# Lacadame/DiffSci

Hardware: AMD Instinct MI355X
Metric: samples/sec (50-step Karras Heun), PUNetG 64ch 128x128 (higher is better)
Workload: dtype f32 (3x3 convs: fp16 hi+lo split, 3 fp16 MFMA products, fp32 accumulate); 1 GPU; PUNetG 64-base-ch, 1x128x128 fields, batch 64 per GPU, 50-step Heun deterministic sampler (99 network evaluations); global_batch=64, parallelism=dp1 (batch shards, all-gather of samples), world_size=1, backend=none (one process), hipgraph=True

## Files before the change

### build.py

```python
#!/usr/bin/env python3
import os
import subprocess
import sys

ROOT = os.path.dirname(os.path.abspath(__file__))
CSRC = os.path.join(ROOT, "diffsci_amd", "csrc")
OUTDIR = os.path.join(ROOT, "diffsci_amd", "_lib")
LIB = os.path.join(OUTDIR, "libdiffsci_hip.so")
SOURCES = ["ds_api.hip", "ds_step.hip", "ds_ddpm.hip", "ds_inpaint.hip", "ds_norm.hip", "ds_gnorm.hip", "ds_normtab.hip", "ds_conv.hip", "ds_conv6.hip", "ds_conv3h.hip", "ds_conv3p.hip", "ds_convup.hip", "ds_conv1h.hip", "ds_conv_s2.hip", "ds_convdirect.hip", "ds_conv3d.hip", "ds_resample.hip", "ds_attn.hip", "ds_attn3h.hip", "ds_small.hip", "ds_amax.hip", "ds_tokens.hip", "ds_convit.hip", "ds_groupnorm.hip", "ds_window.hip", "ds_periodize.hip"]
HIPCC = os.environ.get("HIPCC", "/opt/rocm/bin/hipcc")
FLAGS = ["--offload-arch=gfx950", "-O3", "-ffp-contract=off", "-fPIC", "-std=c++17",
         "-Wall", "-Wno-unused-function"] + os.environ.get("DS_EXTRA_HIPCC_FLAGS", "").split()
EXTRA_FLAGS = {f: ["-fno-slp-vectorize"] for f in ("ds_conv3h.hip", "ds_conv3p.hip", "ds_convup.hip", "ds_conv1h.hip", "ds_conv_s2.hip")}
EXTRA_FLAGS["ds_conv3p.hip"] = EXTRA_FLAGS["ds_conv3p.hip"] + ["-Wno-inline-asm"]


def _stale():
    if not os.path.exists(LIB):
        return True
    t = os.path.getmtime(LIB)
    deps = [os.path.join(CSRC, f) for f in os.listdir(CSRC)] + [os.path.join(ROOT, "include", "diffsci_hip.h"), os.path.abspath(__file__)]
    return any(os.path.getmtime(d) > t for d in deps)


def build(force=False, verbose=True):
    os.makedirs(OUTDIR, exist_ok=True)
    if not force and not _stale():
        return LIB
    objs = []
    procs = []
    for src in SOURCES:
        obj = os.path.join(OUTDIR, src.replace(".hip", ".o"))
        cmd = [HIPCC] + FLAGS + EXTRA_FLAGS.get(src, []) + ["-c", os.path.join(CSRC, src), "-o", obj]
        if verbose:
            print(" ".join(cmd), flush=True)
        procs.append((src, subprocess.Popen(cmd)))
        objs.append(obj)
    for src, p in procs:
        if p.wait() != 0:
            raise RuntimeError(f"hipcc failed on {src}")
    cmd = [HIPCC, "--offload-arch=gfx950", "-shared", "-fPIC", "-o", LIB] + objs
    if verbose:
        print(" ".join(cmd), flush=True)
    subprocess.check_call(cmd)
    return LIB

# ... 4 lines not shown
```

### diffsci_amd/csrc/ds_conv1h.hip

```cpp
#include "ds_common.h"
#include "ds_conv_epilogue.h"
#include "ds_h3_common.h"

namespace {

using ds_epi::f32x16;
using ds_h3::f16x8;
using ds_h3::split2;
using ds_h3::u32x4;
typedef const __attribute__((address_space(1))) float* gfloat_ptr;
typedef const __attribute__((address_space(1))) char* gchar_ptr;
typedef float f32x2 __attribute__((ext_vector_type(2)));
typedef const __attribute__((address_space(1))) f32x2* gfloat2_ptr;

constexpr int COT = 64, NT = 256, KC = 16;
constexpr int NPOS = 256;
constexpr int XBUF_VEC = 2 * 2 * NPOS;
constexpr int WSLAB_VEC = 2 * 2 * COT;
constexpr int NXB = 3, NWS = 3;
constexpr int RING_BYTES = (NXB * XBUF_VEC + NWS * WSLAB_VEC) * 16;
constexpr int EPI_BYTES = 4 * 64 * 2 * 32 * 4;
constexpr int STAGE_BYTES = RING_BYTES > EPI_BYTES ? RING_BYTES : EPI_BYTES;
constexpr int LDS_BYTES = STAGE_BYTES + 128 * 4;
constexpr int TWO_RING_BYTES = (NXB * XBUF_VEC + NWS * 2 * WSLAB_VEC) * 16;
constexpr int TWO_EPI_BYTES = 8 * 64 * 2 * 32 * 4;
static_assert(TWO_EPI_BYTES >= TWO_RING_BYTES, "bias / shift rows behind the larger of the two");
constexpr int LDS_BYTES_TWO = TWO_EPI_BYTES + 2 * 128 * 4;
constexpr int NXCD = 8;

struct Conv1hArgs {
  float* out;
  const float* in;
  const u32x4* wp;
  const float* bias;
  const float* shift;
  const float* res1;
  const float* res2;
  float* tile_stats;
  int res1_up;
  const unsigned* in_amax;
  unsigned* out_amax;
  int wshift;
  int amax_split;
  int shift_stride;
  int B, Cin, Cout, H, W, Hin, Win;
  int tiles_x, tiles_y, n_cot, n_chunks;
  int n_cot_wg;
  unsigned n_blocks;
};

__device__ __forceinline__ void step_barrier() {
  asm volatile("s_waitcnt lgkmcnt(0)\n\ts_barrier" ::: "memory");
}

template <int MODE, bool W16, bool TWO = false>
__global__ __launch_bounds__(TWO ? 2 * NT : NT, 2) void k_conv1h(const Conv1hArgs a) {
  constexpr int TW = W16 ? 16 : 32, TH = W16 ? 16 : 8;
  constexpr int COTS = TWO ? 2 : 1;
  constexpr int KR = TWO ? KC / 2 : KC;
  extern __shared__ __attribute__((aligned(16))) unsigned char smem[];
  u32x4* Xs = reinterpret_cast<u32x4*>(smem);
  u32x4* Ws = Xs + NXB * XBUF_VEC;
  float* BS = reinterpret_cast<float*>(smem + (TWO ? TWO_EPI_BYTES : STAGE_BYTES));
  const int tid = threadIdx.x;
  const int lane = tid & 63;
  const int wv = __builtin_amdgcn_readfirstlane(tid >> 6);
  const int cw = TWO ? wv >> 2 : 0;
  const int wq = wv & 3;
  const int pix = tid & (NT - 1);
  const int li = lane & 31, lh = lane >> 5;

  unsigned bid;
  {
    const unsigned x = blockIdx.x % NXCD, k = blockIdx.x / NXCD;
    const unsigned per = a.n_blocks / NXCD, rem = a.n_blocks % NXCD;
    bid = x * per + (x < rem ? x : rem) + k;
// ... 96 lines not shown
  x_fetch(R1, n > 1 ? 1 : 0);
  __builtin_amdgcn_sched_barrier(0);
  ascale = ds_epi::act_scale_of(amax_bits, a.wshift);
  w_store(W0, 0);
  x_store(R0, 0);
  ds_epi::commit_bias_shift(BS, bias_shift, COTS);
  __syncthreads();

  int buf = 0;
  auto step = [&](float (&Ra)[KR], u32x4& Wa, float (&Rb)[KR], u32x4& Wb, int g) {
    const int gf = g + 2 < n ? g + 2 : n - 1;
    w_fetch(Wa, gf);
    x_fetch(Ra, gf);
    mma(g % NWS, buf);
    const int nb = buf == NXB - 1 ? 0 : buf + 1;
    w_store(Wb, (g + 1) % NWS);
    x_store(Rb, nb);
    buf = nb;
    step_barrier();
  };
  int g = 0;
  for (; g + 1 < n; g += 2) {
    step(R0, W0, R1, W1, g);
    step(R1, W1, R0, W0, g + 1);
  }
  if (g < n) step(R0, W0, R1, W1, g);
  __syncthreads();

  {
    ds_epi::Args e;
    e.out = a.out; e.bias = a.bias; e.shift = a.shift; e.res1 = a.res1; e.res2 = a.res2; e.res1_up = a.res1_up;
    e.unscale = ds_epi::unscale_from_in(ascale.in_scale, a.wshift); e.shift_stride = a.shift_stride;
    e.out_amax = a.out_amax ? a.out_amax + b + ((a.amax_split > 0 && (cot + cw) * COT >= a.amax_split) ? a.B : 0) : nullptr;
    e.b = b; e.co_base = (cot + cw) * COT; e.y0 = y0 + (W16 ? 4 : 2) * wq; e.x0 = x0;
    e.Cout = a.Cout; e.H = a.H; e.W = a.W;
    e.tile_stats = a.tile_stats; e.tile = ty * a.tiles_x + tx; e.ntiles = a.tiles_x * a.tiles_y;
    float* tile = reinterpret_cast<float*>(smem) + wv * (64 * 2 * 32);
    ds_epi::store_tile<W16>(acc, tile, BS + 128 * cw, e);
    if (a.tile_stats) {
      __syncthreads();
      if constexpr (TWO) {
        if (tid < 128) {
          e.co_base = (cot + (tid >> 6)) * COT;
          ds_epi::store_tile_stats(reinterpret_cast<const float*>(smem) + (tid >> 6) * 4 * (64 * 2 * 32), 64 * 2 * 32, e, tid & 63);
        }
      } else {
        ds_epi::store_tile_stats(reinterpret_cast<const float*>(smem), 64 * 2 * 32, e);
      }
    }
  }
}

__global__ void k_pack1h(_Float16* packed, const float* __restrict__ w, int Cout, int Cin, int n_chunks, float scale,
                         size_t total) {
  size_t i = (size_t)blockIdx.x * blockDim.x + threadIdx.x;
  if (i >= total) return;
  size_t t = i;
  const int c8 = t % 8; t /= 8;
  const int co64 = t % COT; t /= COT;
  const int h = t % 2; t /= 2;
  const int piece = t % 2; t /= 2;
  const int chunk = t % n_chunks; t /= n_chunks;
  const int cot = (int)t;
  const int co = cot * COT + co64, ci = chunk * KC + 8 * h + c8;
  float v = 0.f;
  if (co < Cout && ci < Cin) v = w[(size_t)co * Cin + ci] * scale;
  const _Float16 hi = (_Float16)v;
  const _Float16 lo = (_Float16)(v - (float)hi);
  packed[i] = piece == 0 ? hi : lo;
}

inline int conv1h_two() {
  static const int v = [] { const char* e = getenv("DS_CONV1_TWO"); return e ? atoi(e) : 1; }();
// ... 37 lines not shown
  DS_REQUIRE(packed && w, DS_ERR_NULL, "ds_conv1x1_h3_pack_weights: NULL pointer");
  DS_REQUIRE(Cout > 0 && Cin > 0, DS_ERR_SHAPE, "ds_conv1x1_h3_pack_weights: Cout=%d Cin=%d", Cout, Cin);
  DS_REQUIRE(wshift >= -40 && wshift <= 40, DS_ERR_SHAPE, "ds_conv1x1_h3_pack_weights: wshift %d out of range", wshift);
  const int n_chunks = (Cin + KC - 1) / KC;
  const size_t total = ds_conv1x1_h3_packed_bytes(Cout, Cin) / 2;
  hipLaunchKernelGGL(k_pack1h, dim3((unsigned)((total + 255) / 256)), dim3(256), 0, ds::as_stream(stream),
                     reinterpret_cast<_Float16*>(packed), w, Cout, Cin, n_chunks, ldexpf(1.0f, wshift), total);
  DS_CHECK_LAUNCH("ds_conv1x1_h3_pack_weights");
  return DS_OK;
}

int ds_conv1x1_h3(float* out, const float* in, const void* w_packed, int wshift, const float* bias, const float* shift,
                  int shift_stride, const float* res1, const float* res2, int B, int Cin, int Cout, int H, int W,
                  int load_mode, float* tile_stats, const unsigned* in_amax, unsigned* out_amax, int amax_split, void* stream) {
  DS_REQUIRE(out && in && w_packed, DS_ERR_NULL, "ds_conv1x1_h3: NULL pointer");
  DS_REQUIRE(B >= 0 && Cin > 0 && Cout > 0 && H > 0 && W > 0, DS_ERR_SHAPE,
             "ds_conv1x1_h3: bad shape B=%d Cin=%d Cout=%d H=%d W=%d", B, Cin, Cout, H, W);
  DS_REQUIRE(load_mode == DS_LOAD_PLAIN || load_mode == DS_LOAD_UPSAMPLE2 || load_mode == DS_LOAD_AVGPOOL2,
             DS_ERR_UNSUPPORTED, "ds_conv1x1_h3: load_mode %d", load_mode);
  DS_REQUIRE(load_mode != DS_LOAD_UPSAMPLE2 || (H % 2 == 0 && W % 2 == 0), DS_ERR_SHAPE,
             "ds_conv1x1_h3: UPSAMPLE2 needs even output H, W (got %d x %d)", H, W);
  DS_REQUIRE(shift == nullptr || shift_stride == 0 || shift_stride >= Cout, DS_ERR_SHAPE,
             "ds_conv1x1_h3: shift_stride %d < Cout %d", shift_stride, Cout);
  DS_REQUIRE((reinterpret_cast<uintptr_t>(w_packed) & 15u) == 0, DS_ERR_SHAPE, "ds_conv1x1_h3: w_packed must be 16-byte aligned");
  DS_REQUIRE(load_mode != DS_LOAD_AVGPOOL2 || (reinterpret_cast<uintptr_t>(in) & 7u) == 0, DS_ERR_SHAPE,
             "ds_conv1x1_h3: AVGPOOL2 input must be 8-byte aligned");
  DS_REQUIRE(wshift >= -40 && wshift <= 40, DS_ERR_SHAPE, "ds_conv1x1_h3: wshift %d out of range", wshift);
  DS_REQUIRE(amax_split >= 0 && amax_split % COT == 0, DS_ERR_SHAPE, "ds_conv1x1_h3: amax_split %d must be a multiple of 64", amax_split);
  if (B == 0) return DS_OK;
  Conv1hArgs a;
  a.out = out; a.in = in; a.wp = reinterpret_cast<const u32x4*>(w_packed); a.bias = bias; a.shift = shift;
  a.res1 = res1; a.res2 = res2; a.shift_stride = shift_stride; a.tile_stats = tile_stats; a.res1_up = 0;
  a.wshift = wshift; a.in_amax = in_amax; a.out_amax = out_amax; a.amax_split = amax_split;
  a.B = B; a.Cin = Cin; a.Cout = Cout; a.H = H; a.W = W;
  a.Hin = load_mode == DS_LOAD_AVGPOOL2 ? 2 * H : (load_mode == DS_LOAD_UPSAMPLE2 ? H / 2 : H);
  a.Win = load_mode == DS_LOAD_AVGPOOL2 ? 2 * W : (load_mode == DS_LOAD_UPSAMPLE2 ? W / 2 : W);
  DS_REQUIRE((long long)a.Hin * a.Win < (1ll << 29), DS_ERR_SHAPE, "ds_conv1x1_h3: a channel plane exceeds 2^29 floats");
  const long long pad32 = (long long)((W + 31) / 32 * 32) * ((H + 7) / 8 * 8);
  const long long pad16 = (long long)((W + 15) / 16 * 16) * ((H + 15) / 16 * 16);
  const bool w16 = pad16 < pad32;
  const int TW = w16 ? 16 : 32, TH = w16 ? 16 : 8;
  a.tiles_x = (W + TW - 1) / TW; a.tiles_y = (H + TH - 1) / TH;
  a.n_cot = (Cout + COT - 1) / COT;
  a.n_chunks = (Cin + KC - 1) / KC;
  const long long blocks = (long long)B * a.tiles_y * a.tiles_x * a.n_cot;
  DS_REQUIRE(blocks > 0 && blocks < (1ll << 31), DS_ERR_SHAPE, "ds_conv1x1_h3: grid of %lld workgroups is out of range", blocks);
  a.n_blocks = (unsigned)blocks;
  hipStream_t s = ds::as_stream(stream);
  if (w16) {
    if (load_mode == DS_LOAD_PLAIN) return launch_conv1h<DS_LOAD_PLAIN, true>(a, s);
    if (load_mode == DS_LOAD_UPSAMPLE2) return launch_conv1h<DS_LOAD_UPSAMPLE2, true>(a, s);
    return launch_conv1h<DS_LOAD_AVGPOOL2, true>(a, s);
  }
  if (load_mode == DS_LOAD_PLAIN) return launch_conv1h<DS_LOAD_PLAIN, false>(a, s);
  if (load_mode == DS_LOAD_UPSAMPLE2) return launch_conv1h<DS_LOAD_UPSAMPLE2, false>(a, s);
  return launch_conv1h<DS_LOAD_AVGPOOL2, false>(a, s);
}

}
```

### diffsci_amd/csrc/ds_conv3h.hip

```cpp
#include "ds_common.h"
#include <cstring>
#include "ds_conv3h_args.h"

#ifdef DS_STAMP
unsigned long long* g_stamps = nullptr;
#define STAMP_SLOTS 16
#define STAMP_AT(slot) a.stamps[((size_t)(blockIdx.z * gridDim.y + blockIdx.y) * gridDim.x + blockIdx.x) * STAMP_SLOTS + (slot)]
#define STAMP(slot) do { if (threadIdx.x == 0) STAMP_AT(slot) = __builtin_amdgcn_s_memrealtime(); } while (0)
#define STAMP_CLK(slot) do { if (threadIdx.x == 0) STAMP_AT(slot) = __builtin_amdgcn_s_memtime(); } while (0)
#define STAMP_PLACE() do { if (threadIdx.x == 0) { STAMP_AT(8) = __builtin_amdgcn_s_getreg((31 << 11) | 4); STAMP_AT(9) = __builtin_amdgcn_s_getreg((31 << 11) | 20); } } while (0)
#else
#define STAMP(slot) do {} while (0)
#define STAMP_CLK(slot) do {} while (0)
#define STAMP_PLACE() do {} while (0)
#endif

namespace {

using namespace ds_conv3;

template <int MT> struct Frags { f16x8 a[2][MT]; f16x8 b[2][2]; };

template <int MODE, bool W16, bool PRE, bool CIRC, int NW, bool S16 = false, bool IMGIN = false, bool TWO = false, bool VEC = false>
__global__ __launch_bounds__(64 * NW, TWO ? 2 : NW / 2) void k_conv3h(const Conv3hArgs a) {
// ... 678 lines not shown
             "ds_conv2d_h3: MAXPOOL2 input must be 8-byte aligned");
  DS_REQUIRE(wshift >= -40 && wshift <= 40, DS_ERR_SHAPE, "ds_conv2d_h3: wshift %d out of range", wshift);
  DS_REQUIRE(prenorm == nullptr || load_mode != DS_LOAD_MAXPOOL2, DS_ERR_UNSUPPORTED,
             "ds_conv2d_h3: prenorm cannot be combined with the max-pool load (pooling follows the activation)");
  DS_REQUIRE((reinterpret_cast<uintptr_t>(prenorm) & 15u) == 0, DS_ERR_SHAPE, "ds_conv2d_h3: prenorm must be 16-byte aligned");
  if (B == 0) return DS_OK;
  Conv3hArgs a;
  a.prenorm = prenorm; a.tile_stats = tile_stats; a.circular = circular; a.res1_up = res1_up; a.oy = oy; a.ox = ox;
  a.ntiles_magic40 = 0; a.ncot_magic40 = 0; a.pc_prio = 0; a.pc_skew_mask = 0;
  {
    static const int early = [] { const char* e = getenv("DS_CONV_TWO_EARLY"); return e ? atoi(e) : 1; }();
    a.two_early = early;
  }
  a.out = out; a.in = in; a.wp = reinterpret_cast<const u32x4*>(w_packed); a.bias = bias; a.shift = shift;
  a.res1 = res1; a.res2 = res2; a.shift_stride = shift_stride;
  a.wshift = wshift; a.in_amax = in_amax; a.out_amax = out_amax;
  a.pool_out = pool_out;
  a.B = B; a.Cin = Cin; a.Cout = Cout; a.H = H; a.W = W;
  a.Hin = load_mode == DS_LOAD_MAXPOOL2 ? 2 * H : (load_mode == DS_LOAD_UPSAMPLE2 ? H / 2 : H);
  a.Win = load_mode == DS_LOAD_MAXPOOL2 ? 2 * W : (load_mode == DS_LOAD_UPSAMPLE2 ? W / 2 : W);
  DS_REQUIRE((long long)Cin * a.Hin * a.Win < (1ll << 31), DS_ERR_SHAPE, "ds_conv2d_h3: per-sample input exceeds 2^31 floats");
  const long long pad32 = (long long)((W + 31) / 32 * 32) * ((H + 7) / 8 * 8);
  const long long pad16 = (long long)((W + 15) / 16 * 16) * ((H + 15) / 16 * 16);
  const bool w16 = pad16 < pad32;
  const int TW = w16 ? 16 : 32, TH = w16 ? 16 : 8;
  a.tiles_x = (W + TW - 1) / TW; a.tiles_y = (H + TH - 1) / TH;
  a.n_cot = (Cout + COT - 1) / COT;
  a.n_chunks = (Cin + KC - 1) / KC;
  a.tiles_x_magic = a.tiles_x == 1 ? 0u : (unsigned)((1ull << 32) / (unsigned)a.tiles_x) + 1u;
#ifdef DS_STAMP
  a.stamps = g_stamps;
#endif
  hipStream_t s = ds::as_stream(stream);
  if (!w16 && load_mode == DS_LOAD_PLAIN && conv3h_shape16()) {
    bool launched = false;
    const int rc = conv3p_try_launch(a, s, &launched, raw, pooled);
    if (rc != DS_OK || launched) return rc;
  }
#define DS_L3(M, W) (prenorm ? launch_conv3h<M, W, true>(a, s) : launch_conv3h<M, W, false>(a, s))
  if (w16) {
    if (load_mode == DS_LOAD_PLAIN) return DS_L3(DS_LOAD_PLAIN, true);
    if (load_mode == DS_LOAD_MAXPOOL2) return launch_conv3h<DS_LOAD_MAXPOOL2, true, false>(a, s);
    return DS_L3(DS_LOAD_UPSAMPLE2, true);
  }
  if (load_mode == DS_LOAD_PLAIN) return DS_L3(DS_LOAD_PLAIN, false);
  if (load_mode == DS_LOAD_MAXPOOL2) return launch_conv3h<DS_LOAD_MAXPOOL2, false, false>(a, s);
  return DS_L3(DS_LOAD_UPSAMPLE2, false);
#undef DS_L3
}

size_t ds_conv_images_bytes(int B, int C, int H, int W) {
  if (B <= 0 || C <= 0 || H <= 0 || W <= 0) return 0;
  return (size_t)B * ((C + KC - 1) / KC) * 4 * (size_t)(H + 2) * (W + 2) * 16;
}

static int conv2d_h3_img(float* out, const void* images, const void* w_packed, int wshift, const float* bias, const float* shift,
                         int shift_stride, const float* res1, const float* res2, int B, int Cin, int Cout, int H, int W,
                         int flags, float* tile_stats, unsigned* out_amax, void* stream, float* pool_out, bool* pooled) {
  DS_REQUIRE(out && images && w_packed, DS_ERR_NULL, "ds_conv2d_h3_img: NULL pointer");
  DS_REQUIRE((flags & ~DS_RES1_UPSAMPLED) == 0, DS_ERR_UNSUPPORTED, "ds_conv2d_h3_img: flags %d (DS_RES1_UPSAMPLED only)", flags);
  DS_REQUIRE(!(flags & DS_RES1_UPSAMPLED) || (res1 && H % 2 == 0 && W % 2 == 0 && (reinterpret_cast<uintptr_t>(res1) & 7u) == 0),
             DS_ERR_SHAPE, "ds_conv2d_h3_img: RES1_UPSAMPLED needs res1 [B, Cout, H/2, W/2] (8-byte aligned) and even H, W");
  DS_REQUIRE(B >= 0 && Cin > 0 && Cout > 0 && H > 0 && W > 0, DS_ERR_SHAPE,
             "ds_conv2d_h3_img: bad shape B=%d Cin=%d Cout=%d H=%d W=%d", B, Cin, Cout, H, W);
  DS_REQUIRE(((Cin + KC - 1) / KC) % 2 == 0, DS_ERR_UNSUPPORTED,
             "ds_conv2d_h3_img: the image-input kernel is the 16x16x32 variant: an even number of 16-channel chunks (Cin = %d)", Cin);
// ... 76 lines not shown
```

### diffsci_amd/csrc/ds_conv3h_args.h

```cpp
#pragma once
#include "ds_common.h"
#include "ds_conv_epilogue.h"
#include "ds_h3_common.h"

namespace ds_conv3 {

using ds_epi::f32x16;
using ds::f32x4;
using ds_h3::u32x4;
using ds_h3::f16x8;
using ds_h3::split2;
using ds_h3::fast_silu;

constexpr int COT = 64, NT = 256;
constexpr int KC = 16;
template <bool W16> struct Geo {
  static constexpr int TH = W16 ? 16 : 8, TW = W16 ? 16 : 32;
  static constexpr int PH = TH + 2, PW = TW + 2, NPOS = PH * PW;
  static constexpr int XITEMS = 2 * NPOS;
  static constexpr int XBUF_VEC = 2 * 2 * NPOS;
};
constexpr int XBUF_VEC = Geo<false>::XBUF_VEC;
constexpr int HPAD16 = 12;
constexpr int XBUF_VEC16 = XBUF_VEC + 2 * HPAD16;
// ... 12 lines not shown
struct Conv3hArgs {
  float* out;
  const float* in;
  const u32x4* wp;
  const float* bias;
  const float* shift;
  const float* res1;
  const float* res2;
  const float* prenorm;
  float* tile_stats;
  const unsigned* in_amax;
  unsigned* out_amax;
  int wshift;
  int shift_stride;
  int res1_up;
  int circular;
  int oy, ox;
  int B, Cin, Cout, H, W, Hin, Win;
  int tiles_x, tiles_y, n_cot, n_chunks;
  unsigned tiles_x_magic;
  unsigned long long ntiles_magic40, ncot_magic40;
  int pc_prio;
  int pc_skew_mask;
  int two_early;
  float* pool_out;
#ifdef DS_STAMP
  unsigned long long* stamps;
#endif
};


int conv3p_try_launch(const Conv3hArgs& a, hipStream_t s, bool* launched, bool raw = false, bool* pooled = nullptr);
int conv3p_try_launch_img(const Conv3hArgs& a, hipStream_t s, bool* launched, bool* pooled = nullptr);

}
```

### diffsci_amd/csrc/ds_conv_epilogue.h

```cpp
#pragma once
#include <hip/hip_runtime.h>

#include "ds_stream.h"

#ifndef DS_AMAX_EPILOGUE
#define DS_AMAX_EPILOGUE 1
#endif

namespace ds_epi {

using ds::amax4;
using ds::f32x4;
using ds::wave_commit_max_always;
typedef float f32x16 __attribute__((ext_vector_type(16)));

struct Args {
  float* out;
  const float* bias;
  const float* shift;
  const float* res1;
  const float* res2;
  int res1_up;
  float unscale;
  int shift_stride;
  int b, co_base;
  int y0, x0;
  int Cout, H, W;
  float* tile_stats;
  int tile, ntiles;
  int pa, pb;
  unsigned* out_amax;
};

struct ActScale {
  float in_scale;
  float unscale;
  float inv_scale;
};
__device__ __forceinline__ unsigned act_bits(const unsigned* amax, int b) {
  if (!amax) return 0u;
  int z = 0;
  asm volatile("" : "+v"(z));
  return amax[b + z];
}
__device__ __forceinline__ int act_exponent_of(unsigned bits, int lo, int hi) {
  bits = __builtin_amdgcn_readfirstlane(bits);
  const int e = (int)((bits >> 23) & 0xffu);
  const int k = (e == 0 || e == 255) ? 0 : 140 - e;
  return k > hi ? hi : (k < lo ? lo : k);
}
__device__ __forceinline__ float pow2f(int k) { return __builtin_bit_cast(float, (unsigned)(127 + k) << 23); }
__device__ __forceinline__ float mul_pow2(float x, int k) { return __builtin_bit_cast(float, __builtin_bit_cast(unsigned, x) + ((unsigned)k << 23)); }
__device__ __forceinline__ float unscale_from_in(float in_scale, int wshift) {
  return __builtin_bit_cast(float, ((unsigned)(254 - wshift) << 23) - __builtin_bit_cast(unsigned, in_scale));
}
__device__ __forceinline__ float unscale_from_inv(float inv_scale, int wshift) {
  return __builtin_bit_cast(float, __builtin_bit_cast(unsigned, inv_scale) - ((unsigned)wshift << 23));
}
__device__ __forceinline__ ActScale act_scale_of(unsigned bits, int wshift) {
  const int hi = 126 - wshift < 126 ? 126 - wshift : 126, lo = -126 - wshift > -126 ? -126 - wshift : -126;
  const int k = act_exponent_of(bits, lo, hi);
  ActScale s;
  s.in_scale = __builtin_bit_cast(float, (unsigned)(127 + k) << 23);
  s.unscale = __builtin_bit_cast(float, (unsigned)(127 - wshift - k) << 23);
// ... 28 lines not shown
    yq = W16 ? (p4 >> 4) : 0;
    const int r_lane = (lane >> 3) & 1;
    gy_lane = e.y0 + (W16 ? 2 * r_lane + yq : r_lane);
    pix_ok = gy_lane < e.H && gx < e.W;
    const size_t plane = (size_t)e.H * e.W;
    idx_lane = ((size_t)e.b * e.Cout + e.co_base + (lane >> 4)) * plane + (size_t)gy_lane * e.W + gx;
    idx_step = 4 * plane;
  }
};

template <bool W16, int MT>
__device__ __forceinline__ void load_residuals(Residuals<MT>& R, const Args& e) {
  if ((e.W & 3) != 0 || (!e.res1 && !e.res2)) return;
  const int lane = threadIdx.x & 63;
  const RowPlan<W16> rp(e);
#pragma unroll
  for (int j = 0; j < 8 * MT; ++j) {
    const bool ok = rp.pix_ok && (e.co_base + 4 * j + (lane >> 4) < e.Cout);
    const size_t idx = ok ? rp.idx_lane + (size_t)j * rp.idx_step : (size_t)0;
    if (e.res1) {
      if (e.res1_up) {
        const size_t lidx = ok ? (((size_t)e.b * e.Cout + e.co_base + 4 * j + (lane >> 4)) * (e.H >> 1) + (rp.gy_lane >> 1)) * (e.W >> 1) + (rp.gx >> 1) : (size_t)0;
        typedef float f32x2_t __attribute__((ext_vector_type(2)));
        const f32x2_t lo = *reinterpret_cast<const f32x2_t*>(e.res1 + lidx);
        R.r1[j] = f32x4{lo[0], lo[1], 0.f, 0.f};
      } else {
        R.r1[j] = *reinterpret_cast<const f32x4*>(e.res1 + idx);
      }
    }
    if (e.res2) R.r2[j] = *reinterpret_cast<const f32x4*>(e.res2 + idx);
  }
}

template <bool W16, int MT, bool PREFETCHED>
__device__ __forceinline__ void store_tile_rows(float* tile, const Args& e, const Residuals<PREFETCHED ? MT : 0>& R);

template <bool W16 = false, int MT = 2>
__device__ __forceinline__ void store_tile(const f32x16 (&acc)[MT][2], float* tile, const float* bs, const Args& e) {
  const int lane = threadIdx.x & 63;
  const int li = lane & 31, lh = lane >> 5;
  constexpr bool PF = MT == 2;
  Residuals<PF ? MT : 0> R;
  if constexpr (PF) load_residuals<W16, MT>(R, e);
#pragma unroll
  for (int m = 0; m < MT; ++m)
#pragma unroll
    for (int q = 0; q < 16; ++q) {
      const int co = 32 * m + (q & 3) + 8 * (q >> 2) + 4 * lh;
      const float bsv = bs[co] + bs[64 + co];
#pragma unroll
      for (int r = 0; r < 2; ++r) tile[(co * 2 + r) * 32 + li] = __builtin_fmaf(acc[m][r][q], e.unscale, bsv);
    }
  store_tile_rows<W16, MT, PF>(tile, e, R);
}

template <bool W16, int MT = 2>
__device__ __forceinline__ void store_tile16(const f32x4 (&acc)[2 * MT][4], float* tile, const float* bs, const Args& e) {
  const int lane = threadIdx.x & 63;
  const int i = lane & 15, g = lane >> 4;
  const float unscale = e.unscale;
  constexpr bool PF = MT == 2;
  Residuals<PF ? MT : 0> R;
  if constexpr (PF) load_residuals<W16, MT>(R, e);
#pragma unroll
  for (int m = 0; m < 2 * MT; ++m)
#pragma unroll
    for (int q = 0; q < 4; ++q) {
      const int co = 16 * m + 4 * g + q;
      const float bsv = bs[co] + bs[64 + co];
#pragma unroll
      for (int n = 0; n < 4; ++n) tile[(co * 2 + (n >> 1)) * 32 + 16 * (n & 1) + i] = __builtin_fmaf(acc[m][n][q], unscale, bsv);
    }
  store_tile_rows<W16, MT, PF>(tile, e, R);
}

template <bool W16, int MT, bool PREFETCHED>
__device__ __forceinline__ void store_tile_rows(float* tile, const Args& e, const Residuals<PREFETCHED ? MT : 0>& R) {
  const int lane = threadIdx.x & 63;
  const RowPlan<W16> rp(e);
  const int p4 = rp.p4, gx = rp.gx, yq = rp.yq;
  const size_t plane = (size_t)e.H * e.W;
  const bool stats = e.tile_stats != nullptr;
  if ((e.W & 3) == 0) {
    const bool pix_ok = rp.pix_ok;
    const size_t idx_lane = rp.idx_lane, idx_step = rp.idx_step;
    const float cnt_row = stats ? row16_sum(pix_ok ? 4.f : 0.f) : 0.f;
    const bool want_amax = DS_AMAX_EPILOGUE && e.out_amax != nullptr;
    float amax = 0.f;
    float sK[8 * MT], ssum[8 * MT], ssq[8 * MT], scnt[8 * MT];
#pragma unroll
    for (int half = 0; half < 2 * MT; ++half) {
      f32x4 v[4], r1[4], r2[4];
      size_t idx[4];
      bool ok[4];
#pragma unroll
      for (int k = 0; k < 4; ++k) {
        const int j = half * 4 + k;
        const int seg = j * 8 + (lane >> 3);
        const int co = seg >> 1;
        ok[k] = pix_ok && (e.co_base + co < e.Cout);
        idx[k] = ok[k] ? idx_lane + (size_t)j * idx_step : (size_t)0;
        v[k] = *reinterpret_cast<const f32x4*>(&tile[seg * 32 + p4]);
      }
      if constexpr (PREFETCHED) {
        if (e.res1) {
          if (e.res1_up) {
#pragma unroll
            for (int k = 0; k < 4; ++k) { const f32x4 lo = R.r1[half * 4 + k]; r1[k] = f32x4{lo[0], lo[0], lo[1], lo[1]}; }
          } else {
// ... 27 lines not shown
#pragma unroll
        for (int k = 0; k < 4; ++k) r2[k] = *reinterpret_cast<const f32x4*>(e.res2 + idx[k]);
      }
      }
      if (e.res1) {
#pragma unroll
        for (int k = 0; k < 4; ++k) v[k] = v[k] + r1[k];
      }
      if (e.res2) {
#pragma unroll
        for (int k = 0; k < 4; ++k) v[k] = v[k] + r2[k];
      }
#pragma unroll
      for (int k = 0; k < 4; ++k)
        if (ok[k]) *reinterpret_cast<f32x4*>(e.out + idx[k]) = v[k];
      if (want_amax) {
#pragma unroll
        for (int k = 0; k < 4; ++k) amax = ok[k] ? fmaxf(amax, amax4(v[k])) : amax;
      }
      if (stats) {
#pragma unroll
        for (int k = 0; k < 4; ++k) {
          const float K = row16_first(ok[k] ? v[k].x : 0.f);
          const f32x4 d = v[k] - K;
          const float sv = ok[k] ? (d.x + d.y) + (d.z + d.w) : 0.f;
          const float qv = ok[k] ? (d.x * d.x + d.y * d.y) + (d.z * d.z + d.w * d.w) : 0.f;
          sK[half * 4 + k] = K;
          ssum[half * 4 + k] = row16_sum(sv);
          ssq[half * 4 + k] = row16_sum(qv);
          scnt[half * 4 + k] = (e.co_base + ((half * 4 + k) * 4 + (lane >> 4)) < e.Cout) ? cnt_row : 0.f;
        }
      }
    }
    if (want_amax) wave_commit_max_always(e.out_amax, amax);
    if (stats) {
      if ((lane & 15) == 0) {
#pragma unroll
        for (int it = 0; it < 8 * MT; ++it) {
          f32x4 o = {sK[it], ssum[it], ssq[it], scnt[it]};
          *reinterpret_cast<f32x4*>(&tile[4 * (4 * it + (lane >> 4))]) = o;
        }
      }
    }
  } else {
    float amax = 0.f;
    for (int i = lane; i < 32 * MT * 2 * 32; i += 64) {
      const int co = i >> 6, r = (i >> 5) & 1, x = i & 31;
      const int gy = e.y0 + (W16 ? 2 * r + (x >> 4) : r), gxx = e.x0 + (W16 ? (x & 15) : x);
      float v = 0.f;
      const bool okv = e.co_base + co < e.Cout && gy < e.H && gxx < e.W;
      if (okv) {
        const size_t idx = ((size_t)e.b * e.Cout + e.co_base + co) * plane + (size_t)gy * e.W + gxx;
        v = tile[i];
        if (e.res1) v = v + (e.res1_up ? e.res1[(((size_t)e.b * e.Cout + e.co_base + co) * (e.H >> 1) + (gy >> 1)) * (e.W >> 1) + (gxx >> 1)]
                                       : e.res1[idx]);
        if (e.res2) v = v + e.res2[idx];
        e.out[idx] = v;
        amax = fmaxf(amax, __builtin_fabsf(v));
      }
      if (stats) {
        const float K = __shfl(v, 0, 64);
        const float d = okv ? v - K : 0.f;
        float sv = d, qv = d * d, nv = okv ? 1.f : 0.f;
#pragma unroll
        for (int o = 32; o > 0; o >>= 1) { sv += __shfl_xor(sv, o, 64); qv += __shfl_xor(qv, o, 64); nv += __shfl_xor(nv, o, 64); }
        if (lane == 0) { tile[4 * co] = K; tile[4 * co + 1] = sv; tile[4 * co + 2] = qv; tile[4 * co + 3] = nv; }
      }
    }
    if (DS_AMAX_EPILOGUE && e.out_amax) wave_commit_max_always(e.out_amax, amax);
  }
}

template <int MT = 2>
__device__ __forceinline__ void store_tile_stats(const float* tiles, int wave_stride, const Args& e, int t = -1) {
  if (t < 0) t = threadIdx.x;
  if (t < 64 && e.co_base + t < e.Cout) {
    f32x4 p[4];
    const int w0 = MT == 1 ? 4 * (t >> 5) : 0, tl = MT == 1 ? (t & 31) : t;
#pragma unroll
    for (int w = 0; w < 4; ++w) p[w] = *reinterpret_cast<const f32x4*>(&tiles[(w0 + w) * wave_stride + 4 * tl]);
    const float K = p[0][0];
    float S = 0.f, Q = 0.f, n = 0.f;
#pragma unroll
    for (int w = 0; w < 4; ++w) {
      const float dk = p[w][3] > 0.f ? p[w][0] - K : 0.f;
      S += p[w][1] + p[w][3] * dk;
      Q += p[w][2] + 2.f * dk * p[w][1] + p[w][3] * dk * dk;
      n += p[w][3];
    }
    f32x4 o = {K, S, Q, n};
    *reinterpret_cast<f32x4*>(e.tile_stats + (((size_t)e.b * e.Cout + e.co_base + t) * e.ntiles + e.tile) * 4) = o;
  }
}

__device__ __forceinline__ float fetch_bias_shift(const float* bias, const float* shift, int shift_stride, int b, int co_base,
                                                   int Cout, int cots = 1) {
  const int t = threadIdx.x;
  const int co = co_base + (t & 63);
  float v = 0.f;
  if (t < 128 * cots && co < Cout) {
    if ((t & 127) < 64) v = bias ? bias[co] : 0.f;
    else v = shift ? shift[(size_t)b * shift_stride + co] : 0.f;
// ... 9 lines not shown
```

### diffsci_amd/csrc/ds_convdirect.hip

```cpp
#include "ds_common.h"
#include "ds_stream.h"
#include <cstdlib>

namespace {

using ds::f32x4;
typedef float f32x2 __attribute__((ext_vector_type(2)));
constexpr int NT = 256, TH = 16, TW = 64, KCH = 8;
constexpr int PH = TH + 2, PSTR = 68;
constexpr int PATCH = PH * PSTR;

template <int COUT>
__global__ __launch_bounds__(NT) void k_conv_direct(float* out, const float* __restrict__ in, const float* w,
                                                    const float* __restrict__ bias, int Cin, int H, int W,
                                                    int tiles_x, int tiles_y, int circular) {
  __shared__ __attribute__((aligned(16))) float patch[KCH * PATCH];
  const int tid = threadIdx.x;
  int bid = blockIdx.x;
  const int tx = bid % tiles_x; bid /= tiles_x;
  const int ty = bid % tiles_y; bid /= tiles_y;
  const int b = bid;
  const int x0 = tx * TW, y0 = ty * TH;
  const size_t HW = (size_t)H * W;
  const float* in_b = in + (size_t)b * Cin * HW;
// ... 59 lines not shown
      }
#pragma unroll
      for (int co = 0; co < COUT; ++co) {
        cptr wk = wc + ((size_t)co * Cin + (c0 + ch)) * 9;
#pragma unroll
        for (int ky = 0; ky < 3; ++ky)
#pragma unroll
          for (int kx = 0; kx < 3; ++kx) {
            const float wv = wk[ky * 3 + kx];
#pragma unroll
            for (int p = 0; p < 4; ++p) acc[co][p] = __builtin_fmaf(wv, v[ky][p + kx], acc[co][p]);
          }
      }
    }
  }
  const int gy = y0 + row, gx = x0 + c4;
  if (gy < H) {
#pragma unroll
    for (int co = 0; co < COUT; ++co) {
      const float bv = bias ? bias[co] : 0.f;
      float* o = out + ((size_t)b * COUT + co) * HW + (size_t)gy * W + gx;
      if ((W & 3) == 0 && gx + 3 < W) {
        f32x4 r = {acc[co][0] + bv, acc[co][1] + bv, acc[co][2] + bv, acc[co][3] + bv};
        *reinterpret_cast<f32x4*>(o) = r;
      } else {
#pragma unroll
        for (int p = 0; p < 4; ++p)
          if (gx + p < W) o[p] = acc[co][p] + bv;
      }
    }
  }
}

template <int COUT>
__global__ __launch_bounds__(NT, 4) void k_conv_direct_v(float* out, const float* __restrict__ in, const float* w,
                                                      const float* __restrict__ bias, int Cin, int H, int W,
                                                      int tiles_x, int tiles_y, int circular) {
  __shared__ __attribute__((aligned(16))) float patch[KCH * PATCH];
  const int tid = threadIdx.x;
  int bid = blockIdx.x;
  const int tx = bid % tiles_x; bid /= tiles_x;
  const int ty = bid % tiles_y; bid /= tiles_y;
  const int b = bid;
  const int x0 = tx * TW, y0 = ty * TH;
  const size_t HW = (size_t)H * W;
  const float* in_b = in + (size_t)b * Cin * HW;
  const int row = tid >> 4, c4 = (tid & 15) * 4;
  typedef const __attribute__((address_space(4))) float* cptr;
  cptr wc = (cptr)w;

  constexpr int NV = KCH * PH * 16 / NT;
  static_assert(KCH * PH * 16 % NT == 0 && KCH * PH * 2 <= 2 * NT, "staging plan");
  int goff[NV], loff[NV];
  unsigned vok = 0;
#pragma unroll
  for (int k = 0; k < NV; ++k) {
    const int idx = tid + NT * k;
    const int ch = idx / (PH * 16), rem = idx - ch * (PH * 16);
    const int r = rem >> 4, g = rem & 15;
    int gy = y0 + r - 1;
    if (circular & ds::WRAP_H) gy = (gy < 0 ? gy + H : gy) % H;
    const bool ok = gy >= 0 && gy < H;
    goff[k] = ch * (int)HW + (ok ? gy : 0) * W + x0 + 4 * g;
    loff[k] = ch * PATCH + r * PSTR + 1 + 4 * g;
    if (ok) vok |= 1u << k;
  }
  int hgoff[2], hloff[2];
  unsigned hok = 0;
#pragma unroll
  for (int k = 0; k < 2; ++k) {
// ... 59 lines not shown
          for (int kx = 0; kx < 3; ++kx) {
            const float wv = wk[ky * 3 + kx];
#pragma unroll
            for (int p = 0; p < 4; ++p) acc[co][p] = __builtin_fmaf(wv, x[ky][p + kx], acc[co][p]);
          }
      }
    }
  }
  const int gy = y0 + row, gx = x0 + c4;
  if (gy < H) {
#pragma unroll
    for (int co = 0; co < COUT; ++co) {
      const float bv = bias ? bias[co] : 0.f;
      f32x4 r = {acc[co][0] + bv, acc[co][1] + bv, acc[co][2] + bv, acc[co][3] + bv};
      *reinterpret_cast<f32x4*>(out + ((size_t)b * COUT + co) * HW + (size_t)gy * W + gx) = r;
    }
  }
}

}

extern "C" int ds_conv2d_direct(float* out, const float* in, const float* w, const float* bias, int B, int Cin, int Cout,
                                int H, int W, int circular, void* stream) {
  DS_REQUIRE(out && in && w, DS_ERR_NULL, "ds_conv2d_direct: NULL pointer");
  DS_REQUIRE(B >= 0 && Cin > 0 && H > 0 && W > 0, DS_ERR_SHAPE, "ds_conv2d_direct: bad shape");
  DS_REQUIRE(Cout >= 1 && Cout <= 4, DS_ERR_UNSUPPORTED, "ds_conv2d_direct: Cout=%d (1..4 supported)", Cout);
  DS_REQUIRE((reinterpret_cast<uintptr_t>(out) & 15u) == 0, DS_ERR_SHAPE, "ds_conv2d_direct: out must be 16-byte aligned");
  if (circular) {
    const int word = circular;
    circular = (word & ~(DS_PAD_ZERO_H | DS_PAD_ZERO_W)) == 1 ? ds::wrap_axes(DS_PAD_CIRCULAR | (word & ~1), false) : -1;
    DS_REQUIRE(circular > 0, DS_ERR_UNSUPPORTED, "ds_conv2d_direct: circular %d (0, 1, or 1 with DS_PAD_ZERO_H or DS_PAD_ZERO_W)", word);
  }
  if (B == 0) return DS_OK;
  const int tiles_x = (W + TW - 1) / TW, tiles_y = (H + TH - 1) / TH;
  const long long blocks = (long long)B * tiles_x * tiles_y;
  DS_REQUIRE(blocks < (1ll << 31), DS_ERR_SHAPE, "ds_conv2d_direct: grid too large");
  hipStream_t s = ds::as_stream(stream);
  dim3 g((unsigned)blocks), t(NT);
  static const bool vec_on = [] { const char* e = getenv("DS_DIRECT_VEC"); return !(e && atoi(e) == 0); }();
  const bool vec = vec_on && W % TW == 0 && Cin % KCH == 0 && (reinterpret_cast<uintptr_t>(in) & 15u) == 0 && (long long)Cin * H * W < (1ll << 31);
#define L(C) do { if (vec) hipLaunchKernelGGL((k_conv_direct_v<C>), g, t, 0, s, out, in, w, bias, Cin, H, W, tiles_x, tiles_y, circular); \
                  else hipLaunchKernelGGL((k_conv_direct<C>), g, t, 0, s, out, in, w, bias, Cin, H, W, tiles_x, tiles_y, circular); } while (0)
  switch (Cout) { case 1: L(1); break; case 2: L(2); break; case 3: L(3); break; default: L(4); }
#undef L
  DS_CHECK_LAUNCH("ds_conv2d_direct");
  return DS_OK;
}
```

Baseline: 84.83 samples/s.

## Add direct FP32 input-layer conv, per-workgroup amax reduction, and low-tile direct conv

After: 85.24 samples/s, median of 6. About the same (+0.5%).

```diff
diff --git a/build.py b/build.py
--- a/build.py
+++ b/build.py
@@ -7,11 +7,11 @@
 CSRC = os.path.join(ROOT, "diffsci_amd", "csrc")
 OUTDIR = os.path.join(ROOT, "diffsci_amd", "_lib")
 LIB = os.path.join(OUTDIR, "libdiffsci_hip.so")
-SOURCES = ["ds_api.hip", "ds_step.hip", "ds_ddpm.hip", "ds_inpaint.hip", "ds_norm.hip", "ds_gnorm.hip", "ds_normtab.hip", "ds_conv.hip", "ds_conv6.hip", "ds_conv3h.hip", "ds_conv3p.hip", "ds_convup.hip", "ds_conv1h.hip", "ds_conv_s2.hip", "ds_convdirect.hip", "ds_conv3d.hip", "ds_resample.hip", "ds_attn.hip", "ds_attn3h.hip", "ds_small.hip", "ds_amax.hip", "ds_tokens.hip", "ds_convit.hip", "ds_groupnorm.hip", "ds_window.hip", "ds_periodize.hip"]
+SOURCES = ["ds_api.hip", "ds_step.hip", "ds_ddpm.hip", "ds_inpaint.hip", "ds_norm.hip", "ds_gnorm.hip", "ds_normtab.hip", "ds_conv.hip", "ds_conv6.hip", "ds_conv3h.hip", "ds_conv3p.hip", "ds_convin.hip", "ds_convup.hip", "ds_conv1h.hip", "ds_conv_s2.hip", "ds_convdirect.hip", "ds_conv3d.hip", "ds_resample.hip", "ds_attn.hip", "ds_attn3h.hip", "ds_small.hip", "ds_amax.hip", "ds_tokens.hip", "ds_convit.hip", "ds_groupnorm.hip", "ds_window.hip", "ds_periodize.hip"]
 HIPCC = os.environ.get("HIPCC", "/opt/rocm/bin/hipcc")
 FLAGS = ["--offload-arch=gfx950", "-O3", "-ffp-contract=off", "-fPIC", "-std=c++17",
          "-Wall", "-Wno-unused-function"] + os.environ.get("DS_EXTRA_HIPCC_FLAGS", "").split()
-EXTRA_FLAGS = {f: ["-fno-slp-vectorize"] for f in ("ds_conv3h.hip", "ds_conv3p.hip", "ds_convup.hip", "ds_conv1h.hip", "ds_conv_s2.hip")}
+EXTRA_FLAGS = {f: ["-fno-slp-vectorize"] for f in ("ds_conv3h.hip", "ds_conv3p.hip", "ds_convin.hip", "ds_convup.hip", "ds_conv1h.hip", "ds_conv_s2.hip")}
 EXTRA_FLAGS["ds_conv3p.hip"] = EXTRA_FLAGS["ds_conv3p.hip"] + ["-Wno-inline-asm"]
 
 
diff --git a/diffsci_amd/csrc/ds_conv1h.hip b/diffsci_amd/csrc/ds_conv1h.hip
--- a/diffsci_amd/csrc/ds_conv1h.hip
+++ b/diffsci_amd/csrc/ds_conv1h.hip
@@ -1,6 +1,7 @@
 #include "ds_common.h"
 #include "ds_conv_epilogue.h"
 #include "ds_h3_common.h"
+#include <cstdlib>
 
 namespace {
 
@@ -42,6 +43,7 @@
   unsigned* out_amax;
   int wshift;
   int amax_split;
+  int amax_per_wave;
   int shift_stride;
   int B, Cin, Cout, H, W, Hin, Win;
   int tiles_x, tiles_y, n_cot, n_chunks;
@@ -204,13 +206,29 @@
     e.out = a.out; e.bias = a.bias; e.shift = a.shift; e.res1 = a.res1; e.res2 = a.res2; e.res1_up = a.res1_up;
     e.unscale = ds_epi::unscale_from_in(ascale.in_scale, a.wshift); e.shift_stride = a.shift_stride;
     e.out_amax = a.out_amax ? a.out_amax + b + ((a.amax_split > 0 && (cot + cw) * COT >= a.amax_split) ? a.B : 0) : nullptr;
+    e.amax_per_wave = a.amax_per_wave;
     e.b = b; e.co_base = (cot + cw) * COT; e.y0 = y0 + (W16 ? 4 : 2) * wq; e.x0 = x0;
     e.Cout = a.Cout; e.H = a.H; e.W = a.W;
     e.tile_stats = a.tile_stats; e.tile = ty * a.tiles_x + tx; e.ntiles = a.tiles_x * a.tiles_y;
     float* tile = reinterpret_cast<float*>(smem) + wv * (64 * 2 * 32);
-    ds_epi::store_tile<W16>(acc, tile, BS + 128 * cw, e);
+    ds_epi::store_tile<W16, 2, true>(acc, tile, BS + 128 * cw, e);
+    const bool want_amax = DS_AMAX_EPILOGUE && a.out_amax != nullptr && !a.amax_per_wave;
+    if (a.tile_stats) __syncthreads();
+    else if (want_amax) step_barrier();
+    if (want_amax && (tid & (NT - 1)) == 0) {
+      auto tile_max = [&](int ct) {
+        const float* p = reinterpret_cast<const float*>(smem) + 4 * ct * (64 * 2 * 32) + ds_epi::AMAX_AT;
+        return fmaxf(fmaxf(p[0], p[64 * 2 * 32]), fmaxf(p[2 * 64 * 2 * 32], p[3 * 64 * 2 * 32]));
+      };
+      float m = tile_max(cw);
+      bool commit = true;
+      if constexpr (TWO) {
+        const bool split = a.amax_split > 0 && cot * COT < a.amax_split && (cot + 1) * COT >= a.amax_split;
+        if (!split) { commit = cw == 0; if (commit) m = fmaxf(m, tile_max(1)); }
+      }
+      if (commit) atomicMax(e.out_amax, __builtin_bit_cast(unsigned, m));
+    }
     if (a.tile_stats) {
-      __syncthreads();
       if constexpr (TWO) {
         if (tid < 128) {
           e.co_base = (cot + (tid >> 6)) * COT;
@@ -314,6 +332,10 @@
   a.out = out; a.in = in; a.wp = reinterpret_cast<const u32x4*>(w_packed); a.bias = bias; a.shift = shift;
   a.res1 = res1; a.res2 = res2; a.shift_stride = shift_stride; a.tile_stats = tile_stats; a.res1_up = 0;
   a.wshift = wshift; a.in_amax = in_amax; a.out_amax = out_amax; a.amax_split = amax_split;
+  {
+    static const int per_wave = [] { const char* e = getenv("DS_CONV1_AMAX_WG"); return (e && atoi(e) == 0) ? 1 : 0; }();
+    a.amax_per_wave = per_wave;
+  }
   a.B = B; a.Cin = Cin; a.Cout = Cout; a.H = H; a.W = W;
   a.Hin = load_mode == DS_LOAD_AVGPOOL2 ? 2 * H : (load_mode == DS_LOAD_UPSAMPLE2 ? H / 2 : H);
   a.Win = load_mode == DS_LOAD_AVGPOOL2 ? 2 * W : (load_mode == DS_LOAD_UPSAMPLE2 ? W / 2 : W);
diff --git a/diffsci_amd/csrc/ds_conv3h.hip b/diffsci_amd/csrc/ds_conv3h.hip
--- a/diffsci_amd/csrc/ds_conv3h.hip
+++ b/diffsci_amd/csrc/ds_conv3h.hip
@@ -734,6 +734,11 @@
   a.stamps = g_stamps;
 #endif
   hipStream_t s = ds::as_stream(stream);
+  if (!w16 && load_mode == DS_LOAD_PLAIN && Cin <= 4) {
+    bool launched = false;
+    const int rc = convin_try_launch(a, s, &launched);
+    if (rc != DS_OK || launched) return rc;
+  }
   if (!w16 && load_mode == DS_LOAD_PLAIN && conv3h_shape16()) {
     bool launched = false;
     const int rc = conv3p_try_launch(a, s, &launched, raw, pooled);
diff --git a/diffsci_amd/csrc/ds_conv3h_args.h b/diffsci_amd/csrc/ds_conv3h_args.h
--- a/diffsci_amd/csrc/ds_conv3h_args.h
+++ b/diffsci_amd/csrc/ds_conv3h_args.h
@@ -68,5 +68,6 @@
 
 int conv3p_try_launch(const Conv3hArgs& a, hipStream_t s, bool* launched, bool raw = false, bool* pooled = nullptr);
 int conv3p_try_launch_img(const Conv3hArgs& a, hipStream_t s, bool* launched, bool* pooled = nullptr);
+int convin_try_launch(const Conv3hArgs& a, hipStream_t s, bool* launched);
 
 }
diff --git a/diffsci_amd/csrc/ds_conv_epilogue.h b/diffsci_amd/csrc/ds_conv_epilogue.h
--- a/diffsci_amd/csrc/ds_conv_epilogue.h
+++ b/diffsci_amd/csrc/ds_conv_epilogue.h
@@ -30,6 +30,7 @@
   int tile, ntiles;
   int pa, pb;
   unsigned* out_amax;
+  int amax_per_wave;
 };
 
 struct ActScale {
@@ -124,10 +125,16 @@
   }
 }
 
-template <bool W16, int MT, bool PREFETCHED>
+template <bool W16, int MT, bool PREFETCHED, bool AMAX_LDS = false>
 __device__ __forceinline__ void store_tile_rows(float* tile, const Args& e, const Residuals<PREFETCHED ? MT : 0>& R);
 
-template <bool W16 = false, int MT = 2>
+constexpr int AMAX_AT = 64 * 4;
+__device__ __forceinline__ void wave_leave_max(float* tile, float m) {
+  m = ds::wave_max(m);
+  if ((threadIdx.x & 63) == 0) tile[AMAX_AT] = m;
+}
+
+template <bool W16 = false, int MT = 2, bool AMAX_LDS = false>
 __device__ __forceinline__ void store_tile(const f32x16 (&acc)[MT][2], float* tile, const float* bs, const Args& e) {
   const int lane = threadIdx.x & 63;
   const int li = lane & 31, lh = lane >> 5;
@@ -143,7 +150,7 @@
 #pragma unroll
       for (int r = 0; r < 2; ++r) tile[(co * 2 + r) * 32 + li] = __builtin_fmaf(acc[m][r][q], e.unscale, bsv);
     }
-  store_tile_rows<W16, MT, PF>(tile, e, R);
+  store_tile_rows<W16, MT, PF, AMAX_LDS>(tile, e, R);
 }
 
 template <bool W16, int MT = 2>
@@ -166,7 +173,7 @@
   store_tile_rows<W16, MT, PF>(tile, e, R);
 }
 
-template <bool W16, int MT, bool PREFETCHED>
+template <bool W16, int MT, bool PREFETCHED, bool AMAX_LDS>
 __device__ __forceinline__ void store_tile_rows(float* tile, const Args& e, const Residuals<PREFETCHED ? MT : 0>& R) {
   const int lane = threadIdx.x & 63;
   const RowPlan<W16> rp(e);
@@ -260,7 +267,10 @@
         }
       }
     }
-    if (want_amax) wave_commit_max_always(e.out_amax, amax);
+    if (want_amax) {
+      if (AMAX_LDS && !e.amax_per_wave) wave_leave_max(tile, amax);
+      else wave_commit_max_always(e.out_amax, amax);
+    }
     if (stats) {
       if ((lane & 15) == 0) {
 #pragma unroll
@@ -295,7 +305,10 @@
         if (lane == 0) { tile[4 * co] = K; tile[4 * co + 1] = sv; tile[4 * co + 2] = qv; tile[4 * co + 3] = nv; }
       }
     }
-    if (DS_AMAX_EPILOGUE && e.out_amax) wave_commit_max_always(e.out_amax, amax);
+    if (DS_AMAX_EPILOGUE && e.out_amax) {
+      if (AMAX_LDS && !e.amax_per_wave) wave_leave_max(tile, amax);
+      else wave_commit_max_always(e.out_amax, amax);
+    }
   }
 }
 
diff --git a/diffsci_amd/csrc/ds_convdirect.hip b/diffsci_amd/csrc/ds_convdirect.hip
--- a/diffsci_amd/csrc/ds_convdirect.hip
+++ b/diffsci_amd/csrc/ds_convdirect.hip
@@ -115,10 +115,11 @@
   }
 }
 
-template <int COUT>
-__global__ __launch_bounds__(NT, 4) void k_conv_direct_v(float* out, const float* __restrict__ in, const float* w,
+template <int COUT, int TH = 16>
+__global__ __launch_bounds__(16 * TH, 4) void k_conv_direct_v(float* out, const float* __restrict__ in, const float* w,
                                                       const float* __restrict__ bias, int Cin, int H, int W,
                                                       int tiles_x, int tiles_y, int circular) {
+  constexpr int NT = 16 * TH, PH = TH + 2, PATCH = PH * PSTR;
   __shared__ __attribute__((aligned(16))) float patch[KCH * PATCH];
   const int tid = threadIdx.x;
   int bid = blockIdx.x;
@@ -244,14 +245,17 @@
     DS_REQUIRE(circular > 0, DS_ERR_UNSUPPORTED, "ds_conv2d_direct: circular %d (0, 1, or 1 with DS_PAD_ZERO_H or DS_PAD_ZERO_W)", word);
   }
   if (B == 0) return DS_OK;
-  const int tiles_x = (W + TW - 1) / TW, tiles_y = (H + TH - 1) / TH;
+  static const int vec_mode = [] { const char* e = getenv("DS_DIRECT_VEC"); return e ? atoi(e) : 1; }();
+  const bool vec = vec_mode != 0 && W % TW == 0 && Cin % KCH == 0 && (reinterpret_cast<uintptr_t>(in) & 15u) == 0 && (long long)Cin * H * W < (1ll << 31);
+  const bool low = vec && vec_mode == 2;
+  const int th = low ? 8 : TH;
+  const int tiles_x = (W + TW - 1) / TW, tiles_y = (H + th - 1) / th;
   const long long blocks = (long long)B * tiles_x * tiles_y;
   DS_REQUIRE(blocks < (1ll << 31), DS_ERR_SHAPE, "ds_conv2d_direct: grid too large");
   hipStream_t s = ds::as_stream(stream);
-  dim3 g((unsigned)blocks), t(NT);
-  static const bool vec_on = [] { const char* e = getenv("DS_DIRECT_VEC"); return !(e && atoi(e) == 0); }();
-  const bool vec = vec_on && W % TW == 0 && Cin % KCH == 0 && (reinterpret_cast<uintptr_t>(in) & 15u) == 0 && (long long)Cin * H * W < (1ll << 31);
-#define L(C) do { if (vec) hipLaunchKernelGGL((k_conv_direct_v<C>), g, t, 0, s, out, in, w, bias, Cin, H, W, tiles_x, tiles_y, circular); \
+  dim3 g((unsigned)blocks), t(16 * th);
+#define L(C) do { if (low) hipLaunchKernelGGL((k_conv_direct_v<C, 8>), g, t, 0, s, out, in, w, bias, Cin, H, W, tiles_x, tiles_y, circular); \
+                  else if (vec) hipLaunchKernelGGL((k_conv_direct_v<C>), g, t, 0, s, out, in, w, bias, Cin, H, W, tiles_x, tiles_y, circular); \
                   else hipLaunchKernelGGL((k_conv_direct<C>), g, t, 0, s, out, in, w, bias, Cin, H, W, tiles_x, tiles_y, circular); } while (0)
   switch (Cout) { case 1: L(1); break; case 2: L(2); break; case 3: L(3); break; default: L(4); }
 #undef L
diff --git a/diffsci_amd/csrc/ds_convin.hip b/diffsci_amd/csrc/ds_convin.hip
--- /dev/null
+++ b/diffsci_amd/csrc/ds_convin.hip
@@ -0,0 +1,178 @@
+#include "ds_conv3h_args.h"
+#include <cstdlib>
+
+namespace ds_conv3 {
+
+namespace {
+
+constexpr int CW = 16;
+constexpr long long CONVIN_MAX_WGS = 1024;
+
+__device__ __forceinline__ float wave_sum_to_last(float v) {
+  v = ds_epi::row16_sum(v);
+  v += __builtin_bit_cast(float, __builtin_amdgcn_update_dpp(0, __builtin_bit_cast(int, v), 0x142, 0xA, 0xF, false));
+  v += __builtin_bit_cast(float, __builtin_amdgcn_update_dpp(0, __builtin_bit_cast(int, v), 0x143, 0xC, 0xF, false));
+  return v;
+}
+
+struct ConvinArgs {
+  float* out;
+  const float* in;
+  const _Float16* wp;
+  const float* bias;
+  const float* shift;
+  float* tile_stats;
+  unsigned* out_amax;
+  float wunscale;
+  int shift_stride;
+  int circular;
+  int B, Cout, H, W;
+  int tiles_x, ntiles;
+  unsigned items;
+};
+
+template <int CIN>
+__global__ __launch_bounds__(NT) void k_convin(const ConvinArgs a) {
+  constexpr int WROW = (9 * CIN + 3) / 4 * 4;
+  __shared__ __attribute__((aligned(16))) float Wf[COT * WROW];
+  __shared__ unsigned amax_w[2][4];
+  const int tid = threadIdx.x;
+  const int lane = tid & 63;
+  const int wv = __builtin_amdgcn_readfirstlane(tid >> 6);
+  const int cot = blockIdx.y;
+  const int row = lane >> 3, c4 = (lane & 7) * 4;
+
+  for (int i = tid; i < COT * 9 * CIN; i += NT) {
+    const int co = i / (9 * CIN), r = i - co * (9 * CIN);
+    const int ci = r / 9, t = r - ci * 9;
+    const int ky = t / 3, kx = t - ky * 3;
+    const size_t hi = (((((size_t)cot * 3 + ky) * 2 + 0) * 3 + kx) * 2 * COT + co) * 8 + ci;
+    const size_t lo = hi + (size_t)3 * 2 * COT * 8;
+    Wf[co * WROW + r] = ((float)a.wp[hi] + (float)a.wp[lo]) * a.wunscale;
+  }
+  __syncthreads();
+
+  const size_t HW = (size_t)a.H * a.W;
+  const int co0 = cot * COT + wv * CW;
+  const float* wrow = &Wf[wv * CW * WROW];
+  const bool want_amax = a.out_amax != nullptr;
+  const float bias_l = (a.bias && lane < CW) ? a.bias[co0 + lane] : 0.f;
+  unsigned parity = 0;
+
+  for (unsigned item = blockIdx.x; item < a.items; item += gridDim.x) {
+    const int b = (int)(item / (unsigned)a.ntiles), tile = (int)(item - (unsigned)b * (unsigned)a.ntiles);
+    const int ty = tile / a.tiles_x, tx = tile - ty * a.tiles_x;
+    const int gy = ty * 8 + row, gx = tx * 32 + c4;
+
+    float x[CIN][3][6];
+    {
+      int xl = gx - 1, xr = gx + 4;
+      if (a.circular & ds::WRAP_W) { xl = xl < 0 ? xl + a.W : xl; xr = xr >= a.W ? xr - a.W : xr; }
+      const bool okl = xl >= 0, okr = xr < a.W;
+      const float* in_b = a.in + (size_t)b * CIN * HW;
+#pragma unroll
+      for (int ky = 0; ky < 3; ++ky) {
+        int yy = gy + ky - 1;
+        if (a.circular & ds::WRAP_H) yy = yy < 0 ? yy + a.H : (yy >= a.H ? yy - a.H : yy);
+        const bool oky = yy >= 0 && yy < a.H;
+        const float* src = in_b + (size_t)(oky ? yy : 0) * a.W;
+#pragma unroll
+        for (int ci = 0; ci < CIN; ++ci) {
+          const float* p = src + (size_t)ci * HW;
+          const f32x4 m = *reinterpret_cast<const f32x4*>(p + gx);
+          const float l = p[okl ? xl : 0], r = p[okr ? xr : 0];
+          x[ci][ky][0] = (oky && okl) ? l : 0.f;
+          x[ci][ky][1] = oky ? m[0] : 0.f; x[ci][ky][2] = oky ? m[1] : 0.f;
+          x[ci][ky][3] = oky ? m[2] : 0.f; x[ci][ky][4] = oky ? m[3] : 0.f;
+          x[ci][ky][5] = (oky && okr) ? r : 0.f;
+        }
+      }
+    }
+
+    float amax = 0.f;
+    float* o = a.out + ((size_t)b * a.Cout + co0) * HW + (size_t)gy * a.W + gx;
+    float* st = a.tile_stats ? a.tile_stats + (((size_t)b * a.Cout + co0) * a.ntiles + tile) * 4 : nullptr;
+    const float* sh = a.shift ? a.shift + (size_t)b * a.shift_stride + co0 : nullptr;
+    const float shift_l = (sh && lane < CW) ? sh[lane] : 0.f;
+#pragma unroll 2
+    for (int c = 0; c < CW; ++c) {
+      float w[WROW];
+#pragma unroll
+      for (int k = 0; k < WROW / 4; ++k) {
+        const f32x4 t = *reinterpret_cast<const f32x4*>(&wrow[c * WROW + 4 * k]);
+        w[4 * k] = t[0]; w[4 * k + 1] = t[1]; w[4 * k + 2] = t[2]; w[4 * k + 3] = t[3];
+      }
+      float acc[4] = {0.f, 0.f, 0.f, 0.f};
+#pragma unroll
+      for (int ci = 0; ci < CIN; ++ci)
+#pragma unroll
+        for (int ky = 0; ky < 3; ++ky)
+#pragma unroll
+          for (int kx = 0; kx < 3; ++kx)
+#pragma unroll
+            for (int p = 0; p < 4; ++p) acc[p] = __builtin_fmaf(w[ci * 9 + ky * 3 + kx], x[ci][ky][p + kx], acc[p]);
+      f32x4 v = {acc[0], acc[1], acc[2], acc[3]};
+      if (a.bias) v = v + __builtin_bit_cast(float, __builtin_amdgcn_readlane(__builtin_bit_cast(int, bias_l), c));
+      if (sh) v = v + __builtin_bit_cast(float, __builtin_amdgcn_readlane(__builtin_bit_cast(int, shift_l), c));
+      *reinterpret_cast<f32x4*>(o + (size_t)c * HW) = v;
+      if (want_amax) amax = fmaxf(amax, ds::amax4(v));
+      if (st) {
+        const float K = __builtin_bit_cast(float, __builtin_amdgcn_readfirstlane(__builtin_bit_cast(int, v.x)));
+        const f32x4 d = v - K;
+        const float S = wave_sum_to_last((d.x + d.y) + (d.z + d.w));
+        const float Q = wave_sum_to_last((d.x * d.x + d.y * d.y) + (d.z * d.z + d.w * d.w));
+        if (lane == 63) {
+          const f32x4 r = {K, S, Q, 256.f};
+          *reinterpret_cast<f32x4*>(st + (size_t)c * a.ntiles * 4) = r;
+        }
+      }
+    }
+    if (want_amax) {
+      amax = ds::wave_max(amax);
+      if (lane == 0) amax_w[parity][wv] = __builtin_bit_cast(unsigned, amax);
+      asm volatile("s_waitcnt lgkmcnt(0)\n\ts_barrier" ::: "memory");
+      if (tid == 0) {
+        const unsigned m01 = amax_w[parity][0] > amax_w[parity][1] ? amax_w[parity][0] : amax_w[parity][1];
+        const unsigned m23 = amax_w[parity][2] > amax_w[parity][3] ? amax_w[parity][2] : amax_w[parity][3];
+        atomicMax(a.out_amax + b, m01 > m23 ? m01 : m23);
+      }
+      parity ^= 1u;
+    }
+  }
+}
+
+}
+
+static bool convin_on() {
+  static const bool on = [] { const char* e = getenv("DS_CONVIN_DIRECT"); return !(e && atoi(e) == 0); }();
+  return on;
+}
+
+int convin_try_launch(const Conv3hArgs& a, hipStream_t s, bool* launched) {
+  *launched = false;
+  if (!convin_on()) return DS_OK;
+  if (a.Cin > 4 || a.Cout % COT != 0 || a.H % 8 != 0 || a.W % 32 != 0) return DS_OK;
+  if (a.prenorm || a.res1 || a.res2 || a.res1_up || a.pool_out || a.oy != 0 || a.ox != 0 || a.Hin != a.H || a.Win != a.W) return DS_OK;
+  if (((reinterpret_cast<uintptr_t>(a.in) | reinterpret_cast<uintptr_t>(a.out) | reinterpret_cast<uintptr_t>(a.tile_stats)) & 15u) != 0) return DS_OK;
+  const long long items = (long long)a.B * a.tiles_x * a.tiles_y;
+  if (items >= (1ll << 31) || a.n_cot > 65535) return DS_OK;
+  ConvinArgs c;
+  c.out = a.out; c.in = a.in; c.wp = reinterpret_cast<const _Float16*>(a.wp); c.bias = a.bias; c.shift = a.shift;
+  c.tile_stats = a.tile_stats; c.out_amax = a.out_amax;
+  c.wunscale = ldexpf(1.0f, -a.wshift); c.shift_stride = a.shift_stride; c.circular = a.circular;
+  c.B = a.B; c.Cout = a.Cout; c.H = a.H; c.W = a.W;
+  c.tiles_x = a.tiles_x; c.ntiles = a.tiles_x * a.tiles_y; c.items = (unsigned)items;
+  const unsigned gx = (unsigned)(items < CONVIN_MAX_WGS ? items : CONVIN_MAX_WGS);
+  const dim3 g(gx, (unsigned)a.n_cot), t(NT);
+  switch (a.Cin) {
+    case 1: hipLaunchKernelGGL((k_convin<1>), g, t, 0, s, c); break;
+    case 2: hipLaunchKernelGGL((k_convin<2>), g, t, 0, s, c); break;
+    case 3: hipLaunchKernelGGL((k_convin<3>), g, t, 0, s, c); break;
+    default: hipLaunchKernelGGL((k_convin<4>), g, t, 0, s, c); break;
+  }
+  DS_CHECK_LAUNCH("ds_conv2d_h3 (input layer)");
+  *launched = true;
+  return DS_OK;
+}
+
+}
```
